# lis-epfl/multi_agent_pkgs

Hardware: AMD Instinct MI355X
Metric: agent QP-replans/sec (higher is better)
Workload: dtype f64

## Files before the change

multi_agent_pkgs_amd/csrc/hdsm_api.hip:

```cpp
#include <hip/hip_runtime.h>

#include <atomic>
#include <mutex>

#include <cfloat>
#include <rccl/rccl.h>

#include <climits>
#include <cstdio>
#include <cstdlib>
#include <cstring>
#include <new>
#include <string>
#include <vector>

#include "../../include/hdsm.h"
#include "hdsm_consts.h"
#include "hdsm_core.h"
#include "hdsm_level1.h"
#include "hdsm_shapes.h"

namespace {

thread_local std::string g_err;
// ... 93 lines not shown
  run_block<Sol>(reinterpret_cast<typename Sol::S*>(smem), cp, a);
}

__device__ void launch_order_block(int n_inst, const int32_t* __restrict__ key_prev, const int32_t* __restrict__ agent_id, int32_t* __restrict__ order);

struct SetupMapArgs {
  const hdsm::Consts* c;
  const double* state;
  const double* ref;
  double* out;
  int32_t n_inst, N, nk, row_tiles, first_block;
};
__device__ void setup_map_tile(const SetupMapArgs& m, int tile) {
  using v4d = double __attribute__((ext_vector_type(4)));
  const int lane = (int)threadIdx.x & 63;
  const int rt = tile % m.row_tiles, it = tile / m.row_tiles;
  if (it * 16 >= m.n_inst) return;
  const int i = lane & 15, kk = lane >> 4;
  const int row = rt * 16 + i, inst = it * 16 + i, nvt = 9 + 6 * m.N;
  const bool row_on = row < m.nk, inst_on = inst < m.n_inst;
  const double* st = m.state + (int64_t)(inst_on ? inst : 0) * 9;
  const double* rf = m.ref + (int64_t)(inst_on ? inst : 0) * 6 * m.N;
  v4d acc = {0.0, 0.0, 0.0, 0.0};
  constexpr int CH = 9;
  for (int k0 = 0; k0 < nvt; k0 += 4 * CH) {
    double av[CH], bv[CH];
#pragma unroll
    for (int u = 0; u < CH; ++u) {
      const int j = k0 + 4 * u + kk;
      av[u] = (row_on && j < nvt) ? m.c->KT[(int64_t)j * hdsm::KROWS + row] : 0.0;
      bv[u] = (inst_on && j < nvt) ? (j < 9 ? st[j] : rf[j - 9]) : 0.0;
    }
#pragma unroll
    for (int u = 0; u < CH; ++u) acc = __builtin_amdgcn_mfma_f64_16x16x4f64(av[u], bv[u], acc, 0, 0, 0);
  }
  const int col = lane & 15, oi = it * 16 + col;
  if (oi < m.n_inst) {
    for (int r = 0; r < 4; ++r) {
      const int orow = rt * 16 + (lane >> 4) + 4 * r;
      if (orow < m.nk) m.out[(int64_t)oi * hdsm::KROWS + orow] = acc[r];
    }
  }
}

__global__ __launch_bounds__(256) void k_plan_prepass(int N, int n_rob, const double* __restrict__ plans,
                                                      const uint8_t* __restrict__ has_plan, double* __restrict__ pos,
                                                      double* __restrict__ bounds, int n_order, const int32_t* __restrict__ key_prev,
                                                      const int32_t* __restrict__ agent_id, int32_t* __restrict__ order, SetupMapArgs sm) {
  if (sm.out != nullptr && (int)blockIdx.x >= sm.first_block) {
    setup_map_tile(sm, ((int)blockIdx.x - sm.first_block) * 4 + ((int)threadIdx.x >> 6));
    return;
  }
  if (order != nullptr && (int)blockIdx.x == (n_rob + 15) / 16) {
    launch_order_block(n_order, key_prev, agent_id, order);
    return;
  }
  if ((int)blockIdx.x >= (n_rob + 15) / 16) return;
  const int tid = (int)threadIdx.x, i = tid & 15;
  const int k = (int)blockIdx.x * 16 + (tid >> 4);
  const bool live = k < n_rob;
  const bool has = live && has_plan[k];
  const bool on = has && i < N;
  double p[3] = {0.0, 0.0, 0.0};
  if (on) {
    const double* rec = plans + ((int64_t)k * (N + 1) + 1 + i) * 9;
    p[0] = rec[0], p[1] = rec[1], p[2] = rec[2];
  }
  if (live && i < N) {
    double* pk = pos + ((int64_t)k * N + i) * 3;
    pk[0] = p[0], pk[1] = p[1], pk[2] = p[2];
  }
  if (!bounds) return;
  double lo[3], hi[3];
  for (int ax = 0; ax < 3; ++ax) lo[ax] = on ? p[ax] : 1e300, hi[ax] = on ? p[ax] : -1e300;
  for (int off = 8; off > 0; off >>= 1)
    for (int ax = 0; ax < 3; ++ax) {
      lo[ax] = fmin(lo[ax], __shfl_xor(lo[ax], off, 16));
      hi[ax] = fmax(hi[ax], __shfl_xor(hi[ax], off, 16));
    }
  const double cx = 0.5 * (lo[0] + hi[0]), cy = 0.5 * (lo[1] + hi[1]), cz = 0.5 * (lo[2] + hi[2]);
  const double ux = p[0] - cx, uy = p[1] - cy, uz = p[2] - cz;
  double r2 = on ? ux * ux + uy * uy + uz * uz : 0.0;
  bool finite = !on || (r2 == r2);
  for (int off = 8; off > 0; off >>= 1) {
    r2 = fmax(r2, __shfl_xor(r2, off, 16));
    finite = finite && __shfl_xor((int)finite, off, 16);
  }
  if (live && i == 0) {
    double4 out = {0.0, 0.0, 0.0, -1.0};
    if (has) {
      out.x = cx, out.y = cy, out.z = cz;
      out.w = sqrt(r2) * (1.0 + 1e-9);
      if (!finite || !(out.w >= 0.0) || !(out.w < 1e299)) out.w = 1e300;
    }
    *reinterpret_cast<double4*>(bounds + 4 * (int64_t)k) = out;
  }
}

__device__ void launch_order_block(int n_inst, const int32_t* __restrict__ key_prev, const int32_t* __restrict__ agent_id, int32_t* __restrict__ order) {
  __shared__ int bucket[256];
  const int tid = (int)threadIdx.x, nt = (int)blockDim.x;
  for (int b = tid; b < 256; b += nt) bucket[b] = 0;
  __syncthreads();
  for (int k = tid; k < n_inst; k += nt) {
    const int it = key_prev[k];
    atomicAdd(&bucket[255 - (it < 0 ? 0 : (it > 255 ? 255 : it))], 1);
  }
  __syncthreads();
  {
    __shared__ int wave_total[4];
    const int c = bucket[tid & 255];
    int incl = c;
#pragma unroll
    for (int off = 1; off < 64; off <<= 1) {
      const int v = __shfl_up(incl, off, 64);
      if ((tid & 63) >= off) incl += v;
    }
    if ((tid & 63) == 63) wave_total[(tid >> 6) & 3] = incl;
    __syncthreads();
    int base = 0;
    for (int w = 0; w < ((tid >> 6) & 3); ++w) base += wave_total[w];
    if (tid < 256) bucket[tid] = base + incl - c;
  }
  __syncthreads();
  for (int k = tid; k < n_inst; k += nt) {
    const int it = key_prev[k];
    const int slot = atomicAdd(&bucket[255 - (it < 0 ? 0 : (it > 255 ? 255 : it))], 1);
    order[2 * slot] = k, order[2 * slot + 1] = agent_id[k];
  }
}
__global__ __launch_bounds__(256) void k_launch_order(int n_inst, const int32_t* __restrict__ key_prev, const int32_t* __restrict__ agent_id, int32_t* __restrict__ order) {
  launch_order_block(n_inst, key_prev, agent_id, order);
}

__global__ __launch_bounds__(256) void k_publish(int rec, int per, int n_local, const double* __restrict__ traj,
                                                 const uint8_t* __restrict__ has_local, double* __restrict__ out) {
  const int64_t idx = (int64_t)blockIdx.x * blockDim.x + threadIdx.x;
  if (idx >= (int64_t)per * rec) return;
  const int k = (int)(idx / rec), e = (int)(idx % rec);
  const bool has = k < n_local && has_local[k];
  double v = has ? traj[idx] : 0.0;
  if (!has && e == 0) v = __longlong_as_double(0x7ff8000000000000LL);
  out[idx] = v;
}
__global__ __launch_bounds__(256) void k_has_from_sentinel(int rec, int n, const double* __restrict__ plans,
                                                           uint8_t* __restrict__ has) {
  const int k = (int)(blockIdx.x * blockDim.x + threadIdx.x);
  if (k >= n) return;
// ... 391 lines not shown
  hdsm::Args last_args;
  int32_t* h_tree_flag = nullptr;
  int32_t* d_tree_flag = nullptr;
  hdsm::SplitRec* d_recs = nullptr;
  double* d_rec_cand = nullptr;
  long long* d_rec_mw = nullptr;
  int32_t *d_rec_src = nullptr, *d_rec_count = nullptr, *d_items = nullptr;
  int32_t* d_slot_busy = nullptr;
  int32_t *h_item_total = nullptr, *d_item_total = nullptr;
  int32_t *d_split = nullptr, *d_sub_stats = nullptr, *d_sub_warm = nullptr, *d_sub_status = nullptr;
  unsigned long long* d_inc = nullptr;
  int32_t* d_node_pool = nullptr;
  double *d_sub_traj = nullptr, *d_sub_ctrl = nullptr, *d_sub_obj = nullptr, *d_sub_scratch = nullptr;
  uint8_t* d_sub_used = nullptr;
  bool sub_ready = false;
  void* h_out = nullptr;
  size_t h_out_cap = 0;
  double* d_bounds = nullptr;
  double* d_setup = nullptr;
  int setup_mfma = 1;
  double* d_pos = nullptr;
  double* d_rpos = nullptr;
  double* d_rsph = nullptr;
  int32_t* d_order = nullptr;
  int order_min = 0;
  uint8_t* d_zero = nullptr;
  hipEvent_t ev_done = nullptr;
  hipEvent_t ev_k0 = nullptr, ev_k1 = nullptr;
  bool time_kernel = false, timed = false;
  bool launched = false;
  struct Buf {
    void* p = nullptr;
    size_t cap = 0;
  } b_planes, b_common, b_ncommon, b_path, b_cap, b_full, b_pv, b_np;
  hdsm_params prm{};
  hdsm::Consts* d_consts = nullptr;
  double* d_scratch = nullptr;
  int64_t scratch_stride = 0;
  int32_t* d_stats = nullptr;
  long long* d_prof = nullptr;
  int32_t* d_warm = nullptr;
  int32_t *d_agent = nullptr, *d_npoly = nullptr, *d_nrows = nullptr, *d_status = nullptr;
  double *d_state = nullptr, *d_ref = nullptr, *d_A = nullptr, *d_b = nullptr, *d_plans = nullptr;
  double *d_traj = nullptr, *d_ctrl = nullptr, *d_obj = nullptr;
  uint8_t *d_has = nullptr, *d_used = nullptr;
  hipStream_t stream = nullptr;
// ... 115 lines not shown

int launch_rescue(Handle* h, const hdsm::Args& a, hipStream_t st) {
  hdsm::Args r = a;
  r.rescue = 1, r.order = nullptr, r.split_budget = 0, r.item_mode = 0, r.split_info = nullptr, r.inc_bits = nullptr, r.node_pool = nullptr;
  r.tree_flag = nullptr, r.tree_mark = 0, r.warm_out = r.warm, r.ovf_flag = nullptr;
  return launch_shape(h, hdsm::pick_shape(shape_knobs(h), r.n_inst, hdsm::PASS_RESCUE), r, st, r.n_inst);
}

int launch(Handle* h, hdsm::Args a, hipStream_t st) {
  a.scratch = h->d_scratch;
  a.scratch_stride = h->scratch_stride;
  a.st_iters = h->d_stats;
  a.st_nodes = h->d_stats + h->max_inst;
  a.st_sweeps = h->d_stats + 2 * h->max_inst;
  a.st_cand = h->d_stats + 3 * h->max_inst;
  a.st_sph = h->d_stats + 4 * h->max_inst;
  a.st_pairs = h->d_stats + 5 * h->max_inst;
  a.st_flags = reinterpret_cast<uint32_t*>(h->d_stats + 6 * h->max_inst);
  a.st_key = h->d_stats + 7 * h->max_inst;
  a.prof = h->d_prof;
  a.warm = (h->prm.warm_start && a.l1_rows == nullptr) ? h->d_warm : nullptr;
  if (h->launched && st != h->last_stream) HIP_TRY(hipStreamWaitEvent(st, h->ev_done, 0));
  h->last_stream = st;
  a.bounds = nullptr, a.pos = nullptr, a.order = nullptr;
  const bool ordered = a.warm != nullptr && h->order_min > 0 && a.n_inst >= h->order_min;
  if (ordered) a.order = h->d_order;
  const bool packed = h->defer_done && a.l1_rows == nullptr && h->prepass_for == a.plans && h->prepass_n_rob == a.n_rob &&
                      h->prepass_n_inst == a.n_inst && h->prepass_ordered == ordered;
  h->prepass_for = nullptr;
  SetupMapArgs sm{};
  a.setup = nullptr;
  if (a.l1_rows == nullptr && h->setup_mfma && h->d_setup != nullptr) {
    sm.c = h->d_consts, sm.state = a.state, sm.ref = a.ref, sm.out = h->d_setup, sm.n_inst = a.n_inst, sm.N = h->N, sm.nk = 3 * h->n + 12;
    sm.row_tiles = (sm.nk + 15) / 16;
    a.setup = h->d_setup;
  }
  const int sm_blocks = sm.out != nullptr ? (sm.row_tiles * ((a.n_inst + 15) / 16) + 3) / 4 : 0;
  if (packed) {
    a.pos = h->d_pos;
    a.bounds = a.n_rob >= h->bounds_min ? h->d_bounds : nullptr;
    if (sm_blocks > 0) {
      sm.first_block = 0;
      hipLaunchKernelGGL(k_plan_prepass, dim3(sm_blocks), dim3(256), 0, st, h->N, 0, a.plans, a.has_plan, h->d_pos, nullptr, 0, a.st_key, a.agent_id, nullptr, sm);
      HIP_TRY(hipGetLastError());
    }
  } else if (a.l1_rows == nullptr) {
    const bool pre = a.n_rob >= h->bounds_min;
    sm.first_block = (a.n_rob + 15) / 16 + (ordered ? 1 : 0);
    hipLaunchKernelGGL(k_plan_prepass, dim3(sm.first_block + sm_blocks), dim3(256), 0, st, h->N, a.n_rob, a.plans, a.has_plan,
                       h->d_pos, pre ? h->d_bounds : nullptr, a.n_inst, a.st_key, a.agent_id, ordered ? h->d_order : nullptr, sm);
    HIP_TRY(hipGetLastError());
    a.pos = h->d_pos;
    a.bounds = pre ? h->d_bounds : nullptr;
  } else if (ordered) {
    hipLaunchKernelGGL(k_launch_order, dim3(1), dim3(256), 0, st, a.n_inst, a.st_key, a.agent_id, h->d_order);
    HIP_TRY(hipGetLastError());
  }
  int rc;
  if (h->time_kernel) HIP_TRY(hipEventRecord(h->ev_k0, st));
  bool small = false;
  const hdsm::ShapeKnobs knobs = shape_knobs(h);
  auto solve = [&](const hdsm::Args& x, int blocks) -> int {
    const hdsm::Shape s = hdsm::pick_shape(knobs, blocks, hdsm::PASS_ORDINARY);
    small = small || hdsm::SHAPES[s].per_cu > 1;
    return launch_shape(h, s, x, st, blocks);
  };
  a.warm_out = a.warm;
  a.tree_flag = h->d_tree_flag;
  a.ovf_flag = h->d_ovf_flag, a.rescue = 0;
  const bool roomy = a.n_inst <= 2 * h->cus;
  const int budget = h->split_budget > 0 ? h->split_budget : (roomy ? 2 : 8);
  a.tree_mark = budget > hdsm::TREE_MARK ? budget : hdsm::TREE_MARK;
  bool split = h->split_mode == 1;
  if (h->split_mode == 2 && h->h_tree_flag != nullptr) {
    if (*h->h_tree_flag != 0) *h->h_tree_flag = 0, h->split_ttl = 256;
    if (h->split_ttl > 0) split = true, --h->split_ttl;
  }
  const hdsm::Shape items = hdsm::pick_shape(knobs, 0, hdsm::PASS_ITEMS);
  if (split && !h->sub_ready) split = ensure_sub(h, items) == hipSuccess;
  if (!split) {
    rc = solve(a, a.n_inst);
  } else {
    a.split_budget = budget, a.split_info = h->d_split, a.tree_mark = 0;
    a.recs = h->d_recs, a.rec_cand = h->d_rec_cand, a.rec_mw = h->d_rec_mw, a.rec_src = h->d_rec_src, a.rec_count = h->d_rec_count, a.items = h->d_items;
    a.rec_cap = h->rec_cap, a.rows_cap = h->rows_cap, a.items_cap = h->items_cap, a.inc_bits = nullptr, a.node_pool = nullptr, a.item_status = h->d_sub_status;
    const int total_nodes = h->prm.max_nodes > 0 ? h->prm.max_nodes : 2000;
    const int left_nodes = total_nodes - budget > 64 ? total_nodes - budget : 64;
    const int node_cap = left_nodes / 128 > 0 ? left_nodes / 128 : 1;
    a.nodes_pool0 = left_nodes, a.node_cap = node_cap;
    HIP_TRY(hipMemsetAsync(h->d_rec_count, 0, 8 * sizeof(int32_t), st));
    HIP_TRY(hipMemsetAsync(h->d_slot_busy, 0, (size_t)h->pool_cap * sizeof(int32_t), st));
    hdsm::Args a1 = a;
    a1.inc_bits = h->d_inc, a1.node_pool = h->d_node_pool;
    rc = solve(a1, a.n_inst);
    if (rc) return rc;
    hdsm::Args b = a;
    b.item_mode = 1, b.order = nullptr, b.inc_bits = h->d_inc, b.node_pool = h->d_node_pool, b.tree_flag = nullptr;
    b.traj = h->d_sub_traj, b.ctrl = h->d_sub_ctrl, b.used = h->d_sub_used, b.status = h->d_sub_status, b.obj = h->d_sub_obj;
    b.scratch = h->d_sub_scratch, b.warm_out = h->d_sub_warm, b.prof = nullptr, b.pool_cap = h->pool_cap, b.slot_busy = h->d_slot_busy, b.item_total = h->d_item_total;
    b.split_budget = h->item_budget;
    b.split_min = h->item_min > 0 ? h->item_min : (roomy ? 2 : 8);
    b.poll_sleep = h->poll_sleep;
    int32_t* ss = h->d_sub_stats;
    const size_t GI = (size_t)h->items_cap;
    b.st_iters = ss, b.st_nodes = ss + GI, b.st_sweeps = ss + 2 * GI, b.st_cand = ss + 3 * GI, b.st_sph = ss + 4 * GI, b.st_pairs = ss + 5 * GI;
    b.st_flags = reinterpret_cast<uint32_t*>(ss + 6 * GI), b.st_key = ss + 7 * GI;
    small = small || hdsm::SHAPES[items].per_cu > 1;
    int grid = 4096;
    if (h->h_item_total != nullptr && 4 * *h->h_item_total > grid) grid = 4 * *h->h_item_total;
    if (grid > h->items_cap) grid = h->items_cap;
    rc = launch_shape(h, items, b, st, grid);
    if (rc) return rc;
    hipLaunchKernelGGL(k_split_merge, dim3(a.n_inst), dim3(64), 0, st, h->N, h->P, a, b);
    HIP_TRY(hipGetLastError());
  }
  if (rc) return rc;
  h->last_small = small, h->last_args = a;
  if (small && h->h_ovf_flag != nullptr) {
    if (*h->h_ovf_flag != 0) *h->h_ovf_flag = 0, h->rescue_ttl = 256;
    if (h->rescue_ttl > 0) {
// ... 58 lines not shown
                    (void**)&h->d_sub_warm, (void**)&h->d_sub_status, (void**)&h->d_sub_traj, (void**)&h->d_sub_ctrl, (void**)&h->d_sub_obj,
                    (void**)&h->d_sub_used, (void**)&h->d_sub_scratch};
    for (void** p : sub) {
      if (*p) (void)hipFree(*p);
      *p = nullptr;
    }
    (void)hipGetLastError();
    h->split_mode = 0;
  }
  return e;
}

void free_all(Handle* h) {
  void* sub[] = {h->d_recs, h->d_rec_cand, h->d_rec_mw, h->d_rec_src, h->d_rec_count, h->d_items, h->d_slot_busy, h->d_split, h->d_inc, h->d_node_pool, h->d_sub_stats, h->d_sub_warm,
                 h->d_sub_status, h->d_sub_traj, h->d_sub_ctrl, h->d_sub_obj, h->d_sub_used, h->d_sub_scratch};
  for (void* p : sub)
    if (p) (void)hipFree(p);
  if (h->h_tree_flag) (void)hipHostFree(h->h_tree_flag);
  if (h->h_item_total) (void)hipHostFree(h->h_item_total);
  if (h->h_ovf_flag) (void)hipHostFree(h->h_ovf_flag);
  if (h->h_out) (void)hipHostFree(h->h_out);
  void* ptrs[] = {h->d_warm, h->d_prof, h->d_consts, h->d_scratch, h->d_stats, h->d_agent, h->d_npoly, h->d_nrows, h->d_status,
                  h->d_state,  h->d_ref,     h->d_A,     h->d_b,     h->d_plans, h->d_bounds, h->d_setup, h->d_traj,  h->d_ctrl,
                  h->d_obj,    h->d_has,     h->d_used,  h->d_pos,   h->d_rpos,  h->d_rsph,  h->d_zero,  h->d_order, h->b_planes.p, h->b_common.p,
                  h->b_ncommon.p, h->b_path.p, h->b_cap.p, h->b_full.p, h->b_pv.p, h->b_np.p};
  for (void* p : ptrs)
    if (p) (void)hipFree(p);
  if (h->ev_done) (void)hipEventDestroy(h->ev_done);
  if (h->ev_k0) (void)hipEventDestroy(h->ev_k0);
  if (h->ev_k1) (void)hipEventDestroy(h->ev_k1);
  if (h->stream) (void)hipStreamDestroy(h->stream);
}

int check_common(Handle* h, int n_inst, int n_rob) {
  if (!h) return set_err(HDSM_ERR_BAD_ARG, "null handle");
  if (n_inst < 0 || n_rob < 0) return set_err(HDSM_ERR_BAD_ARG, "negative size");
  if (n_inst > h->max_inst) return set_err(HDSM_ERR_CAPACITY, "n_inst exceeds max_instances of the handle");
  if (n_rob > h->n_rob_max) return set_err(HDSM_ERR_CAPACITY, "n_rob exceeds n_rob_max of the handle");
  return HDSM_OK;
}

}

extern "C" {

int32_t hdsm_version(void) { return (1 << 16) | 6; }

// ... 57 lines not shown
    env_int("HDSM_THREADS", 64, 256, &t);
    if (t == 64 || t == 256) h->threads = t;
  }
  h->bounds_min = params->prefilter_min_agents > 0 ? params->prefilter_min_agents : (params->prefilter_min_agents < 0 ? INT_MAX : 256);
  env_int("HDSM_BOUNDS_MIN", 1, INT_MAX, &h->bounds_min);
  {
    hipDeviceProp_t prop;
    const int cus = (hipGetDeviceProperties(&prop, device) == hipSuccess) ? prop.multiProcessorCount : 256;
    h->cus = cus;
    h->duo_min = params->duo_min_instances > 0 ? params->duo_min_instances : (params->duo_min_instances < 0 ? 0 : cus + 1);
    env_int("HDSM_DUO_MIN", 0, INT_MAX, &h->duo_min);
    h->tri_min = h->duo_min > 0 ? 2 * cus + 1 : 0;
    env_int("HDSM_TRI_MIN", 0, INT_MAX, &h->tri_min);
    h->quad_min = h->tri_min > 0 ? 3 * cus + 1 : 0;
    env_int("HDSM_QUAD_MIN", 0, INT_MAX, &h->quad_min);
    env_int("HDSM_SETUP_MFMA", 0, 1, &h->setup_mfma);
    env_int("HDSM_SPLIT", 0, 2, &h->split_mode);
    env_int("HDSM_SPLIT_BUDGET", 1, 100000, &h->split_budget);
    env_int("HDSM_ITEM_BUDGET", 0, 100000, &h->item_budget);
    env_int("HDSM_ITEM_MIN", 1, 100000, &h->item_min);
    env_int("HDSM_POLL_SLEEP", 1, 1000, &h->poll_sleep);
    h->rec_cap = 8 * max_instances < 256 ? 256 : (8 * max_instances > 2048 ? 2048 : 8 * max_instances);
    env_int("HDSM_SPLIT_RECORDS", 1, 1 << 20, &h->rec_cap);
    h->order_min = params->launch_order == 0 ? 2 * cus + 1 : (params->launch_order < 0 ? 0 : params->launch_order);
    env_int("HDSM_ORDER_MIN", 0, INT_MAX, &h->order_min);
  }
  if (params->time_limit_s > 0) {
    int khz = 0;
    if (hipDeviceGetAttribute(&khz, hipDeviceAttributeWallClockRate, device) != hipSuccess || khz <= 0) khz = 100000;
    hc->time_ticks = (long long)(params->time_limit_s * 1e3 * (double)khz);
    if (hc->time_ticks < 1) hc->time_ticks = 1;
  }
  h->scratch_stride = scratch_stride_for(h->n);
  const size_t I = (size_t)max_instances, N = (size_t)h->N, P = (size_t)h->P, RS = (size_t)h->RS;
  hipError_t e = hipSuccess;
  auto ok = [&](hipError_t r) {
    if (e == hipSuccess) e = r;
  };
  for (const ShapeLaunch& l : SHAPE_LAUNCH)
    ok(hipFuncSetAttribute(reinterpret_cast<const void*>(l.kern), hipFuncAttributeMaxDynamicSharedMemorySize, (int)l.shm));
  ok(dmalloc(&h->d_consts, 1));
  ok(dmalloc(&h->d_scratch, I * (size_t)h->scratch_stride));
  ok(dmalloc(&h->d_stats, 8 * I));
  ok(dmalloc(&h->d_warm, (hdsm::MAXNV + 2) * I));
#if defined(HDSM_PROFILE) || defined(HDSM_TIMELINE)
  ok(dmalloc(&h->d_prof, 32 * I));
#endif
  ok(dmalloc(&h->d_agent, I));
  ok(dmalloc(&h->d_npoly, I));
  ok(dmalloc(&h->d_nrows, I * P));
  ok(dmalloc(&h->d_status, I));
  ok(dmalloc(&h->d_state, I * 9));
  ok(dmalloc(&h->d_ref, I * N * 6));
  ok(dmalloc(&h->d_A, I * P * RS * 3));
  ok(dmalloc(&h->d_b, I * P * RS));
  ok(dmalloc(&h->d_plans, (size_t)n_rob_max * (N + 1) * 9));
  ok(dmalloc(&h->d_bounds, (size_t)n_rob_max * 4));
  ok(dmalloc(&h->d_setup, I * hdsm::KROWS));
  ok(dmalloc(&h->d_pos, (size_t)n_rob_max * N * 3));
  ok(dmalloc(&h->d_rpos, (size_t)n_rob_max * (N + 1) * 3));
  ok(dmalloc(&h->d_rsph, (size_t)n_rob_max * 4));
  ok(dmalloc(&h->d_zero, (size_t)n_rob_max));
  ok(dmalloc(&h->d_order, 2 * I));
  ok(dmalloc(&h->d_traj, I * (N + 1) * 9));
  ok(dmalloc(&h->d_ctrl, I * N * 3));
  ok(dmalloc(&h->d_obj, I));
  ok(dmalloc(&h->d_has, (size_t)n_rob_max));
  ok(dmalloc(&h->d_used, I * P));
  if (e == hipSuccess) e = hipHostMalloc(reinterpret_cast<void**>(&h->h_ovf_flag), sizeof(int32_t), hipHostMallocMapped);
  if (e == hipSuccess) {
    *h->h_ovf_flag = 0;
    e = hipHostGetDevicePointer(reinterpret_cast<void**>(&h->d_ovf_flag), h->h_ovf_flag, 0);
  }
  if (e == hipSuccess) e = hipHostMalloc(reinterpret_cast<void**>(&h->h_tree_flag), sizeof(int32_t), hipHostMallocMapped);
  if (e == hipSuccess) {
    *h->h_tree_flag = 0;
    e = hipHostGetDevicePointer(reinterpret_cast<void**>(&h->d_tree_flag), h->h_tree_flag, 0);
  }
  if (e == hipSuccess) e = hipHostMalloc(reinterpret_cast<void**>(&h->h_item_total), sizeof(int32_t), hipHostMallocMapped);
  if (e == hipSuccess) {
    *h->h_item_total = 0;
    e = hipHostGetDevicePointer(reinterpret_cast<void**>(&h->d_item_total), h->h_item_total, 0);
  }
  if (e == hipSuccess) e = hipStreamCreateWithFlags(&h->stream, hipStreamNonBlocking);
  if (e == hipSuccess) e = hipMemcpy(h->d_consts, hc, sizeof *hc, hipMemcpyHostToDevice);
  if (e == hipSuccess) e = hipEventCreateWithFlags(&h->ev_done, hipEventDisableTiming);
// ... 252 lines not shown
                          const double* vel_cap, const double* plans_all, const uint8_t* has_plan,
                          double* ref_full, double* ref, double* path_vel, void* hip_stream) {
  Handle* h = static_cast<Handle*>(handle);
  if (int rc = check_common(h, n_inst, n_rob)) return rc;
  if (n_inst == 0) return HDSM_OK;
  if (!cfg || !agent_id || !path || !n_path || !plans_all || !has_plan || !ref_full || !path_vel || pmax < 1)
    return set_err(HDSM_ERR_BAD_ARG, "null or empty argument");
  HIP_TRY(hipSetDevice(h->device));
  RefArgs a{};
  a.n_inst = n_inst, a.n_rob = n_rob, a.pmax = pmax, a.N = h->N, a.dt = h->prm.dt, a.cfg = *cfg;
  a.agent_id = agent_id, a.path = path, a.n_path = n_path, a.vel_cap = vel_cap, a.plans = plans_all;
  a.has_plan = has_plan, a.ref_full = ref_full, a.ref = ref, a.path_vel = path_vel;
  a.rpos = h->d_rpos, a.rsph = h->d_rsph;
  for (int i = 0; i <= hdsm::MAXH; ++i) {
    double occ = 100 * std::pow(cfg->sens_other_agents, (double)i);
    occ = occ < 0 ? 0 : (occ > 100 ? 100 : occ);
    a.wocc[i] = std::pow(occ / 100, cfg->sens_pot);
  }
  hipStream_t st = static_cast<hipStream_t>(hip_stream);
  if (h->launched && st != h->last_stream) HIP_TRY(hipStreamWaitEvent(st, h->ev_done, 0));
  h->last_stream = st;
  {
    const bool with_pre = h->defer_done;
    const bool ordered = with_pre && h->prm.warm_start && h->order_min > 0 && n_inst >= h->order_min;
    const bool pre = n_rob >= h->bounds_min;
    hipLaunchKernelGGL(k_ref_pack, dim3((n_rob + 15) / 16 + (ordered ? 1 : 0)), dim3(256), 0, st, h->N, n_rob, plans_all, has_plan, h->d_rpos, h->d_rsph,
                       with_pre ? h->d_pos : nullptr, with_pre && pre ? h->d_bounds : nullptr, n_inst, h->d_stats + 7 * h->max_inst, agent_id,
                       ordered ? h->d_order : nullptr);
    h->prepass_for = with_pre ? plans_all : nullptr, h->prepass_n_rob = n_rob, h->prepass_n_inst = n_inst, h->prepass_ordered = ordered;
  }
  HIP_TRY(hipGetLastError());
  if (n_inst >= 256) hipLaunchKernelGGL(k_reference<64>, dim3(n_inst), dim3(64), 0, st, a);
  else hipLaunchKernelGGL(k_reference<256>, dim3(n_inst), dim3(256), 0, st, a);
  HIP_TRY(hipGetLastError());
  if (!h->defer_done) HIP_TRY(hipEventRecord(h->ev_done, st));
  h->launched = true;
  return HDSM_OK;
}

int hdsm_reference(void* handle, const hdsm_ref_config* cfg, int32_t n_inst, int32_t n_rob, const int32_t* agent_id,
                   const double* path, const int32_t* n_path, int32_t pmax, const double* vel_cap,
                   const double* plans_all, const uint8_t* has_plan, double* ref_full, double* ref, double* path_vel) {
  Handle* h = static_cast<Handle*>(handle);
  if (int rc = check_common(h, n_inst, n_rob)) return rc;
  if (n_inst == 0) return HDSM_OK;
  if (!cfg || !agent_id || !path || !n_path || !plans_all || !has_plan || !ref_full || !path_vel || pmax < 1)
    return set_err(HDSM_ERR_BAD_ARG, "null or empty argument");
// ... 312 lines not shown
```

multi_agent_pkgs_amd/csrc/hdsm_core.h:

```cpp
#pragma once
#include <math.h>
#include <stdint.h>

#include <hip/hip_runtime.h>
#define HD __device__ __forceinline__
#define HDN __device__ __noinline__
#define PAR_FOR(i, cnt) for (int i = tid_here(); i < (cnt); i += (int)blockDim.x)
#define HDSM_UNROLL _Pragma("unroll")
#define SYNC() __syncthreads()
#define IS_T0 (HDSM_TX == 0)
namespace hdsm {
__device__ __forceinline__ int atomic_inc_i32(int* p) { return atomicAdd(p, 1); }
__device__ __forceinline__ unsigned tx() {
  unsigned t = threadIdx.x;
#if defined(__HIP_DEVICE_COMPILE__)
  asm volatile("" : "+v"(t));
#endif
  return t;
}
}
#define HDSM_TX (hdsm::tx())
#if defined(__HIP_DEVICE_COMPILE__)
#define HDSM_KERNARG_WORD __attribute__((address_space(4))) long long
#else
// ... 737 lines not shown
        if (vt < 24) {
          const bool lower = vt < 3 || (vt >= 6 && vt < 15);
          s.bnd[vt] = fabs(r.v_b) < ABSENT ? r.v_b : (lower ? -DINF : DINF);
        }
        if (vt < 4 * (MAXH + 1)) (&s.kap[0][0])[vt] = r.v_k;
      };
      ST_PROF(8)
      if (g.warm != nullptr && tid < 64) {
        const int32_t* wp = g.warm + (int64_t)inst * (MAXNV + 2);
        wpre.head = wp[0], wpre.code = tid < MAXNV ? wp[1 + tid] : 0;
      }
      const typename W::LaneReq lane_req = W::init_lane_request(c, tid & 63);
      const int fi0 = tid / 6 + 1, fk0 = tid % 6, fi1 = (tid + 64) / 6 + 1, fk1 = (tid + 64) % 6;
      const double wn0 = c.wn[fk0], wx0 = c.wx[fk0], wn1 = c.wn[fk1], wx1 = c.wx[fk1];
      const int items_inst = max_i(max_i(P * RS, 9 * (N + 1)), max_i(KCOLS + 8, max_i(NV, 4 * (MAXH + 1))));
      constexpr int KC = ((6 * S::LDT > 9 * MAXH ? 6 * S::LDT : 9 * MAXH) + 63) / 64 - 1;
      double cg_late[KC], cu_late[KC];
      HDSM_UNROLL
      for (int u = 0; u < KC; ++u) {
        const int vt = tid + nt * (u + 1), ui = vt / S::LDT, uj = vt % S::LDT;
        cg_late[u] = (vt < 9 * MAXH) ? (&c.g[0][0][0])[vt] : 0.0;
        cu_late[u] = (vt < 6 * S::LDT && ui < 6 && uj < 6) ? c.Ueq[ui * 6 + uj] : 0.0;
      }
      const Req r0 = request(tid);

      ST_PROF(9)
      const bool self_ok = self >= 0 && self < g.n_rob;
      const int sidx = self_ok ? self : 0;
      const uint8_t has_own = g.has_plan[sidx];
      for (int k = tid; k < 3 * N; k += nt) {
        const int ci = k / 3, cax = k % 3;
        const double from_plan = g.plans[((int64_t)sidx * (N + 1) + (ci + 1)) * 9 + cax];
        const double from_state = g.state[(int64_t)inst * 9 + cax];
        s.cprev[ci][cax] = (self_ok && has_own) ? from_plan : from_state;
      }
      ST_PROF(10)
      commit(tid, r0);
      if (g.warm != nullptr && g.l1_rows == nullptr && tid < 64) W::warm_prefetch(g, wpre, tid, self, N);
      ST_PROF(11)
      W::init_lane(R, c, tid & 63, lane_req);
      hrow_own = lane_req.hrow;
      fw0 = (tid < 64) ? ((fi0 == N) ? wn0 : wx0) : 0.0;
      fw1 = (tid < 64) ? ((fi1 == N) ? wn1 : wx1) : 0.0;
      HDSM_UNROLL
      for (int u = 0; u < KC; ++u) {
        const int vt = tid + nt * (u + 1);
        if (vt < 9 * MAXH) {
          (&s.g[0][0][0])[vt] = cg_late[u];
          const int ax = vt / (3 * MAXH), comp = (vt / MAXH) % 3, lag = vt % MAXH;
          s.gz[ax][comp][lag] = 0.0;
          s.gz[ax][comp][MAXH + lag] = (lag < N) ? cg_late[u] : 0.0;
        }
        if (vt < 6 * S::LDT) s.U[vt] = cu_late[u];
      }
      static_assert(6 * S::LDT <= 64 * (KC + 1) && 9 * MAXH <= 64 * (KC + 1), "the late constant items cover the smallest workgroup");
      for (int vt = tid + nt; vt < items_inst; vt += nt) commit(vt, request(vt));
      for (int k = 6 * S::LDT + tid; k < NV * S::LDT; k += nt) s.U[k] = 0.0;
// ... 361 lines not shown
              if (s.assign[i] >= 0) m |= 1ull << (16 * s.assign[i] + i);
            }
          }
          if (m == 0ull) {
            if (!s.have_inc) s.level = 0, s.ng_global = 1;
          } else {
            bool known = false;
            for (int k = 0; k < s.n_nogood; ++k) known = known || (s.nogood[k] & ~m) == 0ull;
            if (!known && s.n_nogood < NOGOODS) s.nogood[s.n_nogood++] = m;
          }
        }
        SYNC();
      }
      const bool lim_before = limit;
      NODE_PROF(21)
      run = select_child(s, c, R, nodes, limit, inst, handed_over, rec_slot);
      NODE_PROF(22)
      if (limit && !lim_before) flags |= FLAG_NODE_LIMIT;
    }

#ifdef HDSM_TIMELINE
    const long long tl_loop_end_ = (long long)wall_clock64();
#endif
#ifdef HDSM_PROFILE
    if (IS_T0 && a.prof) {
      long long* pr = a.prof + (int64_t)inst * 32;
      for (int k = 0; k < 8; ++k) pr[k] = s.prof_acc[k], pr[16 + k] = s.prof_acc[8 + k], pr[24 + k] = s.prof_acc[16 + k];
      pr[8] = t_setup_, pr[9] = t_sweep_, pr[10] = t_leaf_, pr[11] = clock64() - t_begin_;
      pr[12] = iters, pr[13] = sweeps, pr[14] = it_warm_, pr[15] = t_warm_;
    }
#endif
    if (handed_over) {
      SplitRec& rc = a.recs[rec_slot];
      const int lev = s.level, nh = s.ncand, ncl = s.ncold;
      const int64_t rbase = (int64_t)rec_slot * a.rows_cap;
      SYNC();
      PAR_FOR(k, nh + ncl) {
        const int slot = k < nh ? k : CMAX - ncl + (k - nh);
        double* dst = a.rec_cand + (rbase + k) * 4;
        dst[0] = s.cand[slot][0], dst[1] = s.cand[slot][1], dst[2] = s.cand[slot][2], dst[3] = s.cand[slot][3];
        a.rec_mw[rbase + k] = *reinterpret_cast<const long long*>(&s.cand_mw[slot]);
        a.rec_src[rbase + k] = s.cand_src[slot];
      }
      PAR_FOR(k, 3 * (N + 1)) rc.sw_ref[k / 3][k % 3] = s.sw_ref[k / 3][k % 3];
      PAR_FOR(k, s.n_nogood) rc.nogood[k] = s.nogood[k];
      PAR_FOR(k, MAXH) rc.assign[k] = s.assign[k];
// ... 51 lines not shown
          }
          __builtin_amdgcn_s_sleep(1);
        }
        if (in_order) __hip_atomic_store(&a.rec_count[1], first + cnt, __ATOMIC_RELAXED, __HIP_MEMORY_SCOPE_AGENT);
        else atomicExch(&a.rec_count[6], 1);
      }
      if (item >= 0) wg_slot = -1;
    }
    if (IS_T0 && a_in.split_budget > 0 && item < 0)
      a.split_info[2 * inst] = handed_over ? (1 | (s.have_inc ? 2 : 0)) : 0, a.split_info[2 * inst + 1] = handed_over ? rec_slot : -1;
    if (IS_T0 && a.tree_flag != nullptr && a.tree_mark > 0 && nodes >= a.tree_mark) *a.tree_flag = 1;
    const int status = s.have_inc ? (limit ? ST_LIMIT : ST_OPTIMAL) : ST_NO_SOLUTION;
    if (s.have_inc) {
      double* tr = a.traj + (int64_t)out * 9 * (N + 1);
      double* cu = a.ctrl + (int64_t)out * 3 * N;
      PAR_FOR(k, 3 * N) cu[k] = s.inc_x[(k % 3) * N + k / 3];
      PAR_FOR(ax, 3) {
        double xs[3] = {s.state0[ax], s.state0[3 + ax], s.state0[6 + ax]};
        for (int comp = 0; comp < 3; ++comp) s.st[0][3 * comp + ax] = xs[comp];
        for (int i = 0; i < N; ++i) {
          const double u = s.inc_x[ax * N + i];
          double xn[3];
          for (int r = 0; r < 3; ++r)
            xn[r] = c.Ad[ax][r][0] * xs[0] + c.Ad[ax][r][1] * xs[1] + c.Ad[ax][r][2] * xs[2] + c.Bd[ax][r] * u;
          for (int r = 0; r < 3; ++r) {
            xs[r] = xn[r];
            s.st[i + 1][3 * r + ax] = xn[r];
          }
        }
      }
      SYNC();
#ifdef HDSM_TIMELINE
      tl_tail1_ = (long long)wall_clock64();
#endif
      PAR_FOR(k, 9 * (N + 1)) tr[k] = s.st[k / 9][k % 9];
      if (HDSM_TX < 64) {
        const int lane = tid_here();
        double part = (lane < n) ? c.r_u * s.inc_x[lane] * s.inc_x[lane] : 0.0;
        for (int idx = lane; idx < 6 * N; idx += 64) {
          const int i = idx / 6 + 1, k = idx % 6;
          const double e = s.st[i][k] - s.ref[i - 1][k];
          part += ((i == N) ? c.wn[k] : c.wx[k]) * e * e;
        }
        part = wave_sum64(part);
        if (lane == 0) a.obj[out] = part;
      }
      if (IS_T0) {
        uint8_t* us = a.used + (int64_t)out * P;
        for (int j = 0; j < P; ++j) us[j] = 0;
        for (int i = 0; i < N; ++i)
          if (s.inc_assign[i] >= 0 && s.inc_assign[i] < P) us[s.inc_assign[i]] = 1;
      }
    }
#ifdef HDSM_TIMELINE
    tl_tail2_ = (long long)wall_clock64();
#endif
    if (a.warm != nullptr && (!handed_over || s.have_inc)) {
      int32_t* wp = a.warm_out + (int64_t)out * (MAXNV + 2);
      const bool certificate = !s.have_inc && !limit && (item < 0 ? (nodes == 1 || s.ng_global) : s.ng_global != 0) && last_rc == GI_INFEASIBLE && s.q < NV;
      if (certificate) {
        SYNC();
        PAR_FOR(k, NV) {
          const int code = (k < s.q) ? s.act[k] : (k == s.q ? s.inf_id : 0);
          int portable = code;
          if (k <= s.q && id_kind(code) == K_C) {
// ... 155 lines not shown
```

multi_agent_pkgs_amd/csrc/hdsm_shapes.h:

```cpp
#pragma once

#include "hdsm_types.h"

namespace hdsm {
constexpr int CMAX30 = 1536;
constexpr int CMAX48 = 1024;
constexpr int CMAX_DUO = 768;
constexpr int CMAX_TRI = 384;
constexpr int CMAX_QUAD = 256;
constexpr int CMAX_DUO48 = 720;

#define HDSM_SOLVER_SHAPES(X)                                            \
  X(replan30_64, k_replan, 32, hdsm::CMAX30, false, 64, 1)               \
  X(replan30, k_replan, 32, hdsm::CMAX30, false, 256, 1)                 \
  X(replan48_64, k_replan, 48, hdsm::CMAX48, false, 64, 1)               \
  X(replan48, k_replan, 48, hdsm::CMAX48, false, 256, 1)                 \
  X(duo, k_replan_duo, 32, hdsm::CMAX_DUO, false, 256, 2)                \
  X(tri, k_replan_tri, 32, hdsm::CMAX_TRI, false, 128, 3)                \
  X(quad, k_replan_quad, 32, hdsm::CMAX_QUAD, true, 128, 4)              \
  X(duo48, k_replan_duo48, 48, hdsm::CMAX_DUO48, false, 128, 2)

#define HDSM_SHAPE_ENUM(name, kernel, nv, cmax, small, threads, per_cu) SHAPE_##name,
enum Shape : int { HDSM_SOLVER_SHAPES(HDSM_SHAPE_ENUM) NUM_SHAPES };
#undef HDSM_SHAPE_ENUM
// ... 6 lines not shown
#undef HDSM_SHAPE_ROW

struct ShapeKnobs {
  int n, threads, P, RS;
  int duo_min, tri_min, quad_min;
};
enum ShapePass : int {
  PASS_ORDINARY,
  PASS_ITEMS,
  PASS_RESCUE,
};

inline Shape pick_shape(const ShapeKnobs& k, int blocks, ShapePass pass) {
  const bool n30 = k.n <= SPLIT_N_MAX, wide = k.threads == 256;
  const Shape one = n30 ? (k.threads == 64 ? SHAPE_replan30_64 : SHAPE_replan30) : (k.threads == 64 ? SHAPE_replan48_64 : SHAPE_replan48);
  const Shape two = n30 ? SHAPE_duo : SHAPE_duo48;
  if (pass == PASS_RESCUE || !wide) return one;
  if (pass == PASS_ITEMS) return k.duo_min > 0 ? two : one;
  if (n30 && k.quad_min > 0 && blocks >= k.quad_min && k.P <= 4 && k.RS <= 20) return SHAPE_quad;
  if (n30 && k.tri_min > 0 && blocks >= k.tri_min) return SHAPE_tri;
  if (k.duo_min > 0 && blocks >= k.duo_min) return two;
  return one;
}
}
```

multi_agent_pkgs_amd/csrc/hdsm_types.h:

```cpp
#pragma once
#include <stdint.h>

namespace hdsm {

constexpr int MAXH = 16;
constexpr int MAXP = 8;
constexpr int MAXRS = 32;
constexpr int MAXNV = 3 * MAXH;
constexpr int MAXT = 256;
constexpr int KCOLS = 9 + 6 * MAXH;
constexpr int KROWS = 3 * MAXNV + 12;
constexpr int SPLIT_N_MAX = 30;
constexpr int KCH = 3 + 2 * MAXH;
constexpr double ABSENT = 1e20;
constexpr double DINF = 1e300;

struct Consts {
  int32_t N, n, P, RS;
  int32_t max_nodes, max_iters;
  int32_t presweep;
  int32_t leaf_mfma;
  int32_t branch_rule;
  int32_t pick_rule;
  int32_t box_cut;
// ... 55 lines not shown
  const double* b;
  const double* plans;
  const uint8_t* has_plan;
  double* traj;
  double* ctrl;
  uint8_t* used;
  int32_t* status;
  double* obj;
  int32_t* st_iters;
  int32_t* st_nodes;
  int32_t* st_sweeps;
  int32_t* st_cand;
  double* scratch;
  int64_t scratch_stride;
  const double* l1_rows;
  const int32_t* l1_nrows;
  int32_t l1_rmax;
  int32_t* warm;
  long long* prof;
  const double* bounds;
  const double* pos;
  const double* setup;
  const int32_t* order;
  int32_t* st_sph;
  int32_t* st_pairs;
  uint32_t* st_flags;
  int32_t split_budget;
  int32_t split_min;
  int32_t poll_sleep;
  int32_t item_mode;
  int32_t* split_info;
  unsigned long long* inc_bits;
  int32_t node_cap;
  int32_t nodes_pool0;
  int32_t* node_pool;
  SplitRec* recs;
  double* rec_cand;
  long long* rec_mw;
  int32_t* rec_src;
  int32_t* rec_count;
  int32_t pool_cap;
  int32_t* slot_busy;
  int32_t* item_total;
  int32_t* items;
  int32_t* item_status;
  int32_t rec_cap, rows_cap, items_cap;
// ... 10 lines not shown
```

Baseline: 9.566 million.

## Precompute own-plan records in prepass, register-cache order keys and rollout constants

Adds a prepass block group that writes each instance's previous-plan positions into a compact buffer. The solver then loads them with one coalesced read instead of gathering from the plans array inside the timed kernel. Also fully unrolls the setup MFMA loop, keeps launch-order keys in registers between the counting and scatter passes, and caches the rollout and objective constants in registers. Launch ordering now turns on when instances exceed resident slots per CU times CU count. This adds an extra buffer and more register pressure.

New measurement: 9.357 million. 0.978x the previous value.

```diff
diff --git a/multi_agent_pkgs_amd/csrc/hdsm_api.hip b/multi_agent_pkgs_amd/csrc/hdsm_api.hip
--- a/multi_agent_pkgs_amd/csrc/hdsm_api.hip
+++ b/multi_agent_pkgs_amd/csrc/hdsm_api.hip
@@ -139,7 +139,7 @@
   const double* st = m.state + (int64_t)(inst_on ? inst : 0) * 9;
   const double* rf = m.ref + (int64_t)(inst_on ? inst : 0) * 6 * m.N;
   v4d acc = {0.0, 0.0, 0.0, 0.0};
-  constexpr int CH = 9;
+  constexpr int CH = (9 + 6 * hdsm::MAXH + 3) / 4;
   for (int k0 = 0; k0 < nvt; k0 += 4 * CH) {
     double av[CH], bv[CH];
 #pragma unroll
@@ -160,12 +160,39 @@
   }
 }
 
+struct OwnArgs {
+  const double* state;
+  double* out;
+  int32_t n_inst, first_block;
+};
+__device__ void own_record_block(const OwnArgs& o, int blk, int N, int n_rob, const double* __restrict__ plans, const uint8_t* __restrict__ has_plan,
+                                 const int32_t* __restrict__ agent_id) {
+  const int tid = (int)threadIdx.x, i = tid & 15;
+  const int inst = blk * 16 + (tid >> 4);
+  if (inst >= o.n_inst || i >= N) return;
+  const int self = agent_id[inst];
+  const double* sp = o.state + (int64_t)inst * 9;
+  const double s0 = sp[0], s1 = sp[1], s2 = sp[2];
+  const bool self_ok = self >= 0 && self < n_rob;
+  const int sidx = self_ok ? self : 0;
+  const uint8_t has = has_plan[sidx];
+  const double* rec = plans + ((int64_t)sidx * (N + 1) + 1 + i) * 9;
+  const double p0 = rec[0], p1 = rec[1], p2 = rec[2];
+  const bool from_plan = self_ok && has;
+  double* out = o.out + ((int64_t)inst * N + i) * 3;
+  out[0] = from_plan ? p0 : s0, out[1] = from_plan ? p1 : s1, out[2] = from_plan ? p2 : s2;
+}
+
 __global__ __launch_bounds__(256) void k_plan_prepass(int N, int n_rob, const double* __restrict__ plans,
                                                       const uint8_t* __restrict__ has_plan, double* __restrict__ pos,
                                                       double* __restrict__ bounds, int n_order, const int32_t* __restrict__ key_prev,
-                                                      const int32_t* __restrict__ agent_id, int32_t* __restrict__ order, SetupMapArgs sm) {
+                                                      const int32_t* __restrict__ agent_id, int32_t* __restrict__ order, OwnArgs own, SetupMapArgs sm) {
   if (sm.out != nullptr && (int)blockIdx.x >= sm.first_block) {
     setup_map_tile(sm, ((int)blockIdx.x - sm.first_block) * 4 + ((int)threadIdx.x >> 6));
+    return;
+  }
+  if (own.out != nullptr && (int)blockIdx.x >= own.first_block) {
+    own_record_block(own, (int)blockIdx.x - own.first_block, N, n_rob, plans, has_plan, agent_id);
     return;
   }
   if (order != nullptr && (int)blockIdx.x == (n_rob + 15) / 16) {
@@ -179,9 +206,10 @@
   const bool has = live && has_plan[k];
   const bool on = has && i < N;
   double p[3] = {0.0, 0.0, 0.0};
-  if (on) {
+  if (live && i < N) {
     const double* rec = plans + ((int64_t)k * (N + 1) + 1 + i) * 9;
-    p[0] = rec[0], p[1] = rec[1], p[2] = rec[2];
+    const double q0 = rec[0], q1 = rec[1], q2 = rec[2];
+    p[0] = has ? q0 : 0.0, p[1] = has ? q1 : 0.0, p[2] = has ? q2 : 0.0;
   }
   if (live && i < N) {
     double* pk = pos + ((int64_t)k * N + i) * 3;
@@ -219,7 +247,19 @@
   const int tid = (int)threadIdx.x, nt = (int)blockDim.x;
   for (int b = tid; b < 256; b += nt) bucket[b] = 0;
   __syncthreads();
-  for (int k = tid; k < n_inst; k += nt) {
+  constexpr int ORDER_REGS = 16;
+  int bkt[ORDER_REGS], aid[ORDER_REGS];
+#pragma unroll
+  for (int j = 0; j < ORDER_REGS; ++j) {
+    const int k = tid + j * nt;
+    const int it = k < n_inst ? key_prev[k] : 0;
+    aid[j] = k < n_inst ? agent_id[k] : 0;
+    bkt[j] = 255 - (it < 0 ? 0 : (it > 255 ? 255 : it));
+  }
+#pragma unroll
+  for (int j = 0; j < ORDER_REGS; ++j)
+    if (tid + j * nt < n_inst) atomicAdd(&bucket[bkt[j]], 1);
+  for (int k = tid + ORDER_REGS * nt; k < n_inst; k += nt) {
     const int it = key_prev[k];
     atomicAdd(&bucket[255 - (it < 0 ? 0 : (it > 255 ? 255 : it))], 1);
   }
@@ -240,7 +280,15 @@
     if (tid < 256) bucket[tid] = base + incl - c;
   }
   __syncthreads();
-  for (int k = tid; k < n_inst; k += nt) {
+#pragma unroll
+  for (int j = 0; j < ORDER_REGS; ++j) {
+    const int k = tid + j * nt;
+    if (k < n_inst) {
+      const int slot = atomicAdd(&bucket[bkt[j]], 1);
+      order[2 * slot] = k, order[2 * slot + 1] = aid[j];
+    }
+  }
+  for (int k = tid + ORDER_REGS * nt; k < n_inst; k += nt) {
     const int it = key_prev[k];
     const int slot = atomicAdd(&bucket[255 - (it < 0 ? 0 : (it > 255 ? 255 : it))], 1);
     order[2 * slot] = k, order[2 * slot + 1] = agent_id[k];
@@ -678,6 +726,7 @@
   double* d_pos = nullptr;
   double* d_rpos = nullptr;
   double* d_rsph = nullptr;
+  double* d_own = nullptr;
   int32_t* d_order = nullptr;
   int order_min = 0;
   uint8_t* d_zero = nullptr;
@@ -839,8 +888,9 @@
   a.warm = (h->prm.warm_start && a.l1_rows == nullptr) ? h->d_warm : nullptr;
   if (h->launched && st != h->last_stream) HIP_TRY(hipStreamWaitEvent(st, h->ev_done, 0));
   h->last_stream = st;
-  a.bounds = nullptr, a.pos = nullptr, a.order = nullptr;
-  const bool ordered = a.warm != nullptr && h->order_min > 0 && a.n_inst >= h->order_min;
+  a.bounds = nullptr, a.pos = nullptr, a.order = nullptr, a.own = nullptr;
+  const hdsm::ShapeKnobs knobs = shape_knobs(h);
+  const bool ordered = a.warm != nullptr && hdsm::launch_ordered(h->order_min, hdsm::pick_shape(knobs, a.n_inst, hdsm::PASS_ORDINARY), h->cus, a.n_inst);
   if (ordered) a.order = h->d_order;
   const bool packed = h->defer_done && a.l1_rows == nullptr && h->prepass_for == a.plans && h->prepass_n_rob == a.n_rob &&
                       h->prepass_n_inst == a.n_inst && h->prepass_ordered == ordered;
@@ -858,15 +908,18 @@
     a.bounds = a.n_rob >= h->bounds_min ? h->d_bounds : nullptr;
     if (sm_blocks > 0) {
       sm.first_block = 0;
-      hipLaunchKernelGGL(k_plan_prepass, dim3(sm_blocks), dim3(256), 0, st, h->N, 0, a.plans, a.has_plan, h->d_pos, nullptr, 0, a.st_key, a.agent_id, nullptr, sm);
+      hipLaunchKernelGGL(k_plan_prepass, dim3(sm_blocks), dim3(256), 0, st, h->N, 0, a.plans, a.has_plan, h->d_pos, nullptr, 0, a.st_key, a.agent_id, nullptr,
+                         OwnArgs{}, sm);
       HIP_TRY(hipGetLastError());
     }
   } else if (a.l1_rows == nullptr) {
     const bool pre = a.n_rob >= h->bounds_min;
-    sm.first_block = (a.n_rob + 15) / 16 + (ordered ? 1 : 0);
+    OwnArgs own{a.state, h->d_own, a.n_inst, (a.n_rob + 15) / 16 + (ordered ? 1 : 0)};
+    sm.first_block = own.first_block + (a.n_inst + 15) / 16;
     hipLaunchKernelGGL(k_plan_prepass, dim3(sm.first_block + sm_blocks), dim3(256), 0, st, h->N, a.n_rob, a.plans, a.has_plan,
-                       h->d_pos, pre ? h->d_bounds : nullptr, a.n_inst, a.st_key, a.agent_id, ordered ? h->d_order : nullptr, sm);
+                       h->d_pos, pre ? h->d_bounds : nullptr, a.n_inst, a.st_key, a.agent_id, ordered ? h->d_order : nullptr, own, sm);
     HIP_TRY(hipGetLastError());
+    a.own = h->d_own;
     a.pos = h->d_pos;
     a.bounds = pre ? h->d_bounds : nullptr;
   } else if (ordered) {
@@ -876,7 +929,6 @@
   int rc;
   if (h->time_kernel) HIP_TRY(hipEventRecord(h->ev_k0, st));
   bool small = false;
-  const hdsm::ShapeKnobs knobs = shape_knobs(h);
   auto solve = [&](const hdsm::Args& x, int blocks) -> int {
     const hdsm::Shape s = hdsm::pick_shape(knobs, blocks, hdsm::PASS_ORDINARY);
     small = small || hdsm::SHAPES[s].per_cu > 1;
@@ -912,7 +964,7 @@
     rc = solve(a1, a.n_inst);
     if (rc) return rc;
     hdsm::Args b = a;
-    b.item_mode = 1, b.order = nullptr, b.inc_bits = h->d_inc, b.node_pool = h->d_node_pool, b.tree_flag = nullptr;
+    b.item_mode = 1, b.order = nullptr, b.own = nullptr, b.inc_bits = h->d_inc, b.node_pool = h->d_node_pool, b.tree_flag = nullptr;
     b.traj = h->d_sub_traj, b.ctrl = h->d_sub_ctrl, b.used = h->d_sub_used, b.status = h->d_sub_status, b.obj = h->d_sub_obj;
     b.scratch = h->d_sub_scratch, b.warm_out = h->d_sub_warm, b.prof = nullptr, b.pool_cap = h->pool_cap, b.slot_busy = h->d_slot_busy, b.item_total = h->d_item_total;
     b.split_budget = h->item_budget;
@@ -1017,7 +1069,7 @@
   if (h->h_out) (void)hipHostFree(h->h_out);
   void* ptrs[] = {h->d_warm, h->d_prof, h->d_consts, h->d_scratch, h->d_stats, h->d_agent, h->d_npoly, h->d_nrows, h->d_status,
                   h->d_state,  h->d_ref,     h->d_A,     h->d_b,     h->d_plans, h->d_bounds, h->d_setup, h->d_traj,  h->d_ctrl,
-                  h->d_obj,    h->d_has,     h->d_used,  h->d_pos,   h->d_rpos,  h->d_rsph,  h->d_zero,  h->d_order, h->b_planes.p, h->b_common.p,
+                  h->d_obj,    h->d_has,     h->d_used,  h->d_pos,   h->d_rpos,  h->d_rsph,  h->d_zero,  h->d_order, h->d_own, h->b_planes.p, h->b_common.p,
                   h->b_ncommon.p, h->b_path.p, h->b_cap.p, h->b_full.p, h->b_pv.p, h->b_np.p};
   for (void* p : ptrs)
     if (p) (void)hipFree(p);
@@ -1121,7 +1173,7 @@
     env_int("HDSM_POLL_SLEEP", 1, 1000, &h->poll_sleep);
     h->rec_cap = 8 * max_instances < 256 ? 256 : (8 * max_instances > 2048 ? 2048 : 8 * max_instances);
     env_int("HDSM_SPLIT_RECORDS", 1, 1 << 20, &h->rec_cap);
-    h->order_min = params->launch_order == 0 ? 2 * cus + 1 : (params->launch_order < 0 ? 0 : params->launch_order);
+    h->order_min = params->launch_order == 0 ? hdsm::ORDER_BY_RESIDENCY : (params->launch_order < 0 ? 0 : params->launch_order);
     env_int("HDSM_ORDER_MIN", 0, INT_MAX, &h->order_min);
   }
   if (params->time_limit_s > 0) {
@@ -1161,6 +1213,7 @@
   ok(dmalloc(&h->d_rsph, (size_t)n_rob_max * 4));
   ok(dmalloc(&h->d_zero, (size_t)n_rob_max));
   ok(dmalloc(&h->d_order, 2 * I));
+  ok(dmalloc(&h->d_own, I * N * 3));
   ok(dmalloc(&h->d_traj, I * (N + 1) * 9));
   ok(dmalloc(&h->d_ctrl, I * N * 3));
   ok(dmalloc(&h->d_obj, I));
@@ -1459,7 +1512,8 @@
   h->last_stream = st;
   {
     const bool with_pre = h->defer_done;
-    const bool ordered = with_pre && h->prm.warm_start && h->order_min > 0 && n_inst >= h->order_min;
+    const bool ordered = with_pre && h->prm.warm_start &&
+                         hdsm::launch_ordered(h->order_min, hdsm::pick_shape(shape_knobs(h), n_inst, hdsm::PASS_ORDINARY), h->cus, n_inst);
     const bool pre = n_rob >= h->bounds_min;
     hipLaunchKernelGGL(k_ref_pack, dim3((n_rob + 15) / 16 + (ordered ? 1 : 0)), dim3(256), 0, st, h->N, n_rob, plans_all, has_plan, h->d_rpos, h->d_rsph,
                        with_pre ? h->d_pos : nullptr, with_pre && pre ? h->d_bounds : nullptr, n_inst, h->d_stats + 7 * h->max_inst, agent_id,
diff --git a/multi_agent_pkgs_amd/csrc/hdsm_core.h b/multi_agent_pkgs_amd/csrc/hdsm_core.h
--- a/multi_agent_pkgs_amd/csrc/hdsm_core.h
+++ b/multi_agent_pkgs_amd/csrc/hdsm_core.h
@@ -783,17 +783,25 @@
         cg_late[u] = (vt < 9 * MAXH) ? (&c.g[0][0][0])[vt] : 0.0;
         cu_late[u] = (vt < 6 * S::LDT && ui < 6 && uj < 6) ? c.Ueq[ui * 6 + uj] : 0.0;
       }
+      static_assert(3 * MAXH <= 64, "one entry of Args::own per thread");
+      const bool own_pre = g.own != nullptr;
+      double own_v = 0.0;
+      if (own_pre && tid < 3 * N) own_v = g.own[(int64_t)inst * 3 * N + tid];
       const Req r0 = request(tid);
 
       ST_PROF(9)
-      const bool self_ok = self >= 0 && self < g.n_rob;
-      const int sidx = self_ok ? self : 0;
-      const uint8_t has_own = g.has_plan[sidx];
-      for (int k = tid; k < 3 * N; k += nt) {
-        const int ci = k / 3, cax = k % 3;
-        const double from_plan = g.plans[((int64_t)sidx * (N + 1) + (ci + 1)) * 9 + cax];
-        const double from_state = g.state[(int64_t)inst * 9 + cax];
-        s.cprev[ci][cax] = (self_ok && has_own) ? from_plan : from_state;
+      if (own_pre) {
+        if (tid < 3 * N) (&s.cprev[0][0])[tid] = own_v;
+      } else {
+        const bool self_ok = self >= 0 && self < g.n_rob;
+        const int sidx = self_ok ? self : 0;
+        const uint8_t has_own = g.has_plan[sidx];
+        for (int k = tid; k < 3 * N; k += nt) {
+          const int ci = k / 3, cax = k % 3;
+          const double from_plan = g.plans[((int64_t)sidx * (N + 1) + (ci + 1)) * 9 + cax];
+          const double from_state = g.state[(int64_t)inst * 9 + cax];
+          s.cprev[ci][cax] = (self_ok && has_own) ? from_plan : from_state;
+        }
       }
       ST_PROF(10)
       commit(tid, r0);
@@ -1201,6 +1209,16 @@
 #ifdef HDSM_TIMELINE
     const long long tl_loop_end_ = (long long)wall_clock64();
 #endif
+    double rb_ad[3][3], rb_bd[3], rb_ru, rb_w[2];
+    {
+      const int t = tid_here(), ax = t < 3 ? t : 0;
+      for (int r = 0; r < 3; ++r) rb_ad[r][0] = c.Ad[ax][r][0], rb_ad[r][1] = c.Ad[ax][r][1], rb_ad[r][2] = c.Ad[ax][r][2], rb_bd[r] = c.Bd[ax][r];
+      rb_ru = c.r_u;
+      for (int u = 0; u < 2; ++u) {
+        const int idx = (t & 63) + 64 * u, i = idx / 6 + 1, k = idx % 6;
+        rb_w[u] = (i == N) ? c.wn[k] : c.wx[k];
+      }
+    }
 #ifdef HDSM_PROFILE
     if (IS_T0 && a.prof) {
       long long* pr = a.prof + (int64_t)inst * 32;
@@ -1298,7 +1316,7 @@
           const double u = s.inc_x[ax * N + i];
           double xn[3];
           for (int r = 0; r < 3; ++r)
-            xn[r] = c.Ad[ax][r][0] * xs[0] + c.Ad[ax][r][1] * xs[1] + c.Ad[ax][r][2] * xs[2] + c.Bd[ax][r] * u;
+            xn[r] = rb_ad[r][0] * xs[0] + rb_ad[r][1] * xs[1] + rb_ad[r][2] * xs[2] + rb_bd[r] * u;
           for (int r = 0; r < 3; ++r) {
             xs[r] = xn[r];
             s.st[i + 1][3 * r + ax] = xn[r];
@@ -1312,11 +1330,16 @@
       PAR_FOR(k, 9 * (N + 1)) tr[k] = s.st[k / 9][k % 9];
       if (HDSM_TX < 64) {
         const int lane = tid_here();
-        double part = (lane < n) ? c.r_u * s.inc_x[lane] * s.inc_x[lane] : 0.0;
-        for (int idx = lane; idx < 6 * N; idx += 64) {
-          const int i = idx / 6 + 1, k = idx % 6;
-          const double e = s.st[i][k] - s.ref[i - 1][k];
-          part += ((i == N) ? c.wn[k] : c.wx[k]) * e * e;
+        static_assert(6 * MAXH <= 128, "two terms of the objective per lane");
+        double part = (lane < n) ? rb_ru * s.inc_x[lane] * s.inc_x[lane] : 0.0;
+        HDSM_UNROLL
+        for (int u = 0; u < 2; ++u) {
+          const int idx = lane + 64 * u;
+          if (idx < 6 * N) {
+            const int i = idx / 6 + 1, k = idx % 6;
+            const double e = s.st[i][k] - s.ref[i - 1][k];
+            part += rb_w[u] * e * e;
+          }
         }
         part = wave_sum64(part);
         if (lane == 0) a.obj[out] = part;
diff --git a/multi_agent_pkgs_amd/csrc/hdsm_shapes.h b/multi_agent_pkgs_amd/csrc/hdsm_shapes.h
--- a/multi_agent_pkgs_amd/csrc/hdsm_shapes.h
+++ b/multi_agent_pkgs_amd/csrc/hdsm_shapes.h
@@ -52,4 +52,11 @@
   if (k.duo_min > 0 && blocks >= k.duo_min) return two;
   return one;
 }
+
+constexpr int ORDER_BY_RESIDENCY = -1;
+inline bool launch_ordered(int order_min, Shape s, int cus, int n_inst) {
+  if (order_min == 0) return false;
+  if (order_min > 0) return n_inst >= order_min;
+  return (long long)n_inst > (long long)SHAPES[s].per_cu * cus;
 }
+}
diff --git a/multi_agent_pkgs_amd/csrc/hdsm_types.h b/multi_agent_pkgs_amd/csrc/hdsm_types.h
--- a/multi_agent_pkgs_amd/csrc/hdsm_types.h
+++ b/multi_agent_pkgs_amd/csrc/hdsm_types.h
@@ -101,6 +101,7 @@
   const double* pos;
   const double* setup;
   const int32_t* order;
+  const double* own;
   int32_t* st_sph;
   int32_t* st_pairs;
   uint32_t* st_flags;
```
